# foolwood/SiamMask

Measured on AMD Instinct MI355X. Metric: frames/sec (255x255 search, 127x127 template), higher is better.
Workload: dtype f16; 1 GPU; siammask_sharp track_mask+track_refine, B=8 streams per GPU in lock-step, cached template; BASELINE configs[2]; variant=sharp, batch_per_gpu=8, global_batch=8, parallelism=streams sharded x1, weights=synthetic_damped (calibrated random init), graph=True, fallbacks=0

## Files before the change

siammask_amd/_lib.py:

```python
import ctypes
import os
import subprocess

import torch

_HERE = os.path.dirname(os.path.abspath(__file__))
LIB_PATH = os.environ.get("SMK_LIB") or os.path.join(_HERE, "libsiammask_hip.so")
CSRC = os.path.join(_HERE, "csrc")

DTYPE = {"f32": 0, "fp32": 0, "float32": 0, "f16": 1, "fp16": 1, "float16": 1, "half": 1,
         "f16x3": 2}
VARIANT = {"rpn": 0, "base": 1, "sharp": 2}
TRACK_BOX, TRACK_MASK, TRACK_NO_MASK_HEAD = 0, 1, 2
HP_STRIDE = 4

SYMBOLS = (
    "smk_version", "smk_last_error", "smk_create", "smk_destroy", "smk_set_weight",
    "smk_finalize_weights", "smk_template", "smk_track", "smk_refine", "smk_set_decode_params", "smk_decode", "smk_step", "smk_set_graph_mode", "smk_seq_status", "smk_seq_sync_check", "smk_set_result_ring", "smk_result_ring_cursor", "smk_set_pipeline", "smk_pipeline_join", "smk_pipeline_observe",
    "smk_debug_read", "smk_debug_seq_inject", "smk_tune", "smk_tune_get", "smk_profile", "smk_profile_dump", "smk_op_conv2d_ex", "smk_op_conv2d", "smk_op_dw_xcorr",
    "smk_op_maxpool3x3s2", "smk_op_stem_pool", "smk_op_l1_block", "smk_op_conv_seq", "smk_host_conv2d_ex", "smk_host_plan_conv", "smk_host_plan_seq", "smk_host_arena_elems", "smk_bench_conv", "smk_packed_size", "smk_export_packed",
    "smk_import_packed", "smk_crop_resize", "smk_paste_mask", "smk_paste_labels", "smk_mask_rbox_workspace", "smk_mask_rbox",
    "smk_trk_state_bytes", "smk_trk_set", "smk_trk_plan", "smk_trk_advance", "smk_crop_resize_dev", "smk_paste_mask_dev",
    "smk_vos_score", "smk_vos_score_dev", "smk_host_trk_plan", "smk_host_trk_advance",
    "smk_vos_score_ex", "smk_vos_score_dev_ex", "smk_label_rects", "smk_frame_sums", "smk_trk_start", "smk_crop_exemplar_dev",
    "smk_host_trk_start", "smk_vot_overlap", "smk_host_vot_overlap",
    "smk_crop_resize_dev_v", "smk_crop_exemplar_dev_v", "smk_frame_sums_v", "smk_trk_start_v", "smk_host_trk_start_v",
    "smk_paste_mask_dev_v", "smk_vot_overlap_dev",
    "smk_set_stream_hp", "smk_trk_advance_hp", "smk_host_trk_advance_hp",
    "smk_iou_score", "smk_iou_score_dev",
    "smk_mask_rbox_workspace_ex", "smk_mask_rbox_ex", "smk_test_mask_rbox_paths",
    "smk_rle_workspace", "smk_rle_encode", "smk_paste_rle_dev", "smk_test_rle_encode",
    "smk_paste_rle_dev_v", "smk_rle_encode_v", "smk_test_rle_encode_v",
    "smk_labels_rle_encode", "smk_vos_rle", "smk_vos_rle_dev",
    "smk_vos_rle_v", "smk_vos_rle_dev_v", "smk_vos_score_v", "smk_vos_score_dev_v",
    "smk_png_worst_bytes", "smk_png_workspace", "smk_png_encode", "smk_host_png_encode", "smk_vos_png_v", "smk_vos_png_dev_v",
# ... 83 lines not shown
    L.smk_tune_get.argtypes = [ctypes.c_char_p, ctypes.POINTER(ci)]
    L.smk_profile.argtypes = [vp, ci]
    L.smk_profile_dump.argtypes = [vp, ctypes.c_char_p, ci]
    ip = ctypes.POINTER(ci)
    L.smk_debug_read.argtypes = [vp, ctypes.c_char_p, fp, ip, ip, ip, vp]
    gp = ctypes.POINTER(ConvGeom)
    L.smk_op_conv2d_ex.argtypes = [ci, ci, gp, fp, fp, fp, fp, vp, fp, vp]
    L.smk_op_conv2d.argtypes = [ci, ci, fp, ci, ci, ci, ci, fp, fp, ci, ci, ci, ci, ci, ci, fp, fp, vp]
    L.smk_op_dw_xcorr.argtypes = [ci, fp, fp, ci, ci, ci, ci, ci, ci, fp, vp]
    L.smk_op_maxpool3x3s2.argtypes = [ci, fp, ci, ci, ci, ci, fp, vp]
    L.smk_op_stem_pool.argtypes = [fp, fp, fp, ci, ci, fp, fp, vp]
    L.smk_op_l1_block.argtypes = [fp] * 9 + [ci, ci, ci, fp, vp]
    L.smk_host_conv2d_ex.argtypes = [gp, fp, fp, fp, fp, vp, fp]
    L.smk_host_plan_conv.argtypes = [gp, ci, ci, ip, ip, ip, ip]
    L.smk_host_arena_elems.argtypes = [ci, ci, ci, ctypes.POINTER(ctypes.c_uint64)]
    L.smk_packed_size.argtypes = [vp, ctypes.POINTER(ctypes.c_uint64)]
    L.smk_export_packed.argtypes = [vp, vp, ctypes.c_uint64]
    L.smk_import_packed.argtypes = [vp, vp, ctypes.c_uint64]
    L.smk_crop_resize.argtypes = [vp, ctypes.c_int64, ci, ci, vp, vp, ci, ci, fp, vp]
    L.smk_paste_mask.argtypes = [fp, ci, vp, ci, ci, ci, ctypes.c_float, ctypes.c_float, vp, fp, vp]
    L.smk_paste_labels.argtypes = [fp, ci, vp, ci, ci, ci, ctypes.c_float, ctypes.c_float, vp, vp]
    L.smk_mask_rbox_workspace.argtypes = [ci, ci, ci]
    L.smk_mask_rbox.argtypes = [vp, ci, ci, ci, ctypes.c_double, vp, ctypes.c_size_t, vp, vp]
    L.smk_mask_rbox_workspace_ex.argtypes = [ci, ci, ci, ci]
    L.smk_mask_rbox_ex.argtypes = [vp, ci, ci, ci, ctypes.c_double, ci, vp, ctypes.c_size_t, vp, vp]
    L.smk_test_mask_rbox_paths.argtypes = [vp, ci, ci, ci, ci, vp]
    cp = ctypes.POINTER(TrkCfg)
    L.smk_trk_state_bytes.argtypes = [ci]
    L.smk_trk_set.argtypes = [vp, ci, vp, vp, vp, ci, ci, vp]
    L.smk_trk_plan.argtypes = [vp, ci, cp, vp]
# ... 108 lines not shown
```

siammask_amd/csrc/conv_igemm.hip:

```cpp
#include <hip/hip_runtime.h>
#include "smk_kernels.h"

namespace smk {

typedef _Float16 half8 __attribute__((ext_vector_type(8)));
typedef _Float16 half4 __attribute__((ext_vector_type(4)));
typedef float floatx16 __attribute__((ext_vector_type(16)));
typedef float floatx4 __attribute__((ext_vector_type(4)));

template <typename T> struct Traits;
template <> struct Traits<float> {
    static constexpr int VE = 4;
    typedef floatx4 frag_t;
    typedef floatx4 out4_t;
    static __device__ inline void mma(floatx16 &acc, const frag_t &a, const frag_t &b) {
        acc = __builtin_amdgcn_mfma_f32_32x32x2f32(a[0], b[0], acc, 0, 0, 0);
        acc = __builtin_amdgcn_mfma_f32_32x32x2f32(a[1], b[1], acc, 0, 0, 0);
        acc = __builtin_amdgcn_mfma_f32_32x32x2f32(a[2], b[2], acc, 0, 0, 0);
        acc = __builtin_amdgcn_mfma_f32_32x32x2f32(a[3], b[3], acc, 0, 0, 0);
    }
    static __device__ inline floatx4 load4(const float *p) { return *(const floatx4 *)p; }
    static __device__ inline void store4(float *p, floatx4 v) { *(floatx4 *)p = v; }
    static constexpr int EV = 4;
    static __device__ inline void loadv(const float *p, float (&v)[4]) {
// ... 826 lines not shown
    hipStream_t s = (hipStream_t)stream;
    const int ch = dtype == DT_F16 ? 64 : 32;
    if (!conv_halo_eligible(p, dtype, bm)) return 1;
    const int ch_n = p.Ci / ch;
    const long wgs64 = (long)p.B * ((p.Ho * p.Wo + 63) / 64) * ((p.Nst + 127) / 128);
    const bool db = bm == 64 && g_tune.halo_db && ch_n >= 2 && wgs64 <= 256;
    if (dtype == DT_F16) {
        if (bm == 128) return launch_halo_t<_Float16, 2, 2, 1, HALO_AROWS_128, 2, 1>(p, s);
        return db ? launch_halo_t<_Float16, 1, 2, 2, HALO_AROWS_64, 3, 2>(p, s) : launch_halo_t<_Float16, 1, 2, 2, HALO_AROWS_64, 3, 1>(p, s);
    }
    if (bm == 128) return launch_halo_t<float, 2, 2, 1, HALO_AROWS_128, 2, 1>(p, s);
    return db ? launch_halo_t<float, 1, 2, 2, HALO_AROWS_64, 3, 2>(p, s) : launch_halo_t<float, 1, 2, 2, HALO_AROWS_64, 3, 1>(p, s);
}

}
namespace smk {
#include "refine_chain_body.inc"
#include "mask_head_tile.inc"
constexpr int CM_CONV_LDS = IgemmLds<2, 2, 1, 128, 2>::v;
constexpr int CM_LDS = CMax<RC_LDS, 2 * CM_CONV_LDS>::v;
static_assert(MH_LDS <= CM_LDS, "the stationary-pixel mask-head tile fits the fused launch's LDS");

__global__ __launch_bounds__(1024) void chain_mask_kernel(const RefineChainParams rp, const ConvBatch cb, const int mh_nsplit) {
    __shared__ __attribute__((aligned(16))) unsigned char smem[CM_LDS];
    if ((int)blockIdx.x < rp.B) {
        refine_chain_body<false>(rp, (int)blockIdx.x, smem);
    } else if (mh_nsplit > 0) {
        mask_head_tile(cb.p[0], (int)blockIdx.x - rp.B, mh_nsplit, smem);
    } else {
        const int half = threadIdx.x >> 9;
        const int bx = 2 * ((int)blockIdx.x - rp.B) + half;
        if (bx < cb.start[cb.n])
            conv_igemm_body<_Float16, 2, 2, 1, 128, OUT_NCHW_F32, 2>(cb, bx, 0, half * 512, smem + half * CM_CONV_LDS);
    }
    if (rp.tail_sem) {
        __syncthreads();
        if (threadIdx.x == 0) {
            const unsigned prev = __hip_atomic_fetch_add(rp.tail_sem + 5, 1u, __ATOMIC_RELAXED, __HIP_MEMORY_SCOPE_AGENT);
            if (prev == gridDim.x - 1) {
                __hip_atomic_store(rp.tail_sem + 5, 0u, __ATOMIC_RELAXED, __HIP_MEMORY_SCOPE_AGENT);
                __hip_atomic_fetch_add(rp.tail_sem, 1u, __ATOMIC_RELEASE, __HIP_MEMORY_SCOPE_AGENT);
            }
        }
    }
}

// ... 5 lines not shown

bool mask_head_eligible(const ConvParams &p, int dtype) {
    return dtype == DT_F16 && p.out_mode == OUT_NCHW_F32 && p.wgt_frag != nullptr && p.kh == 1 && p.kw == 1 && p.stride == 1 &&
           p.stride_x == 1 && p.pad == 0 && !p.ups && !p.pos && p.org_y == 0 && p.org_x == 0 && p.Hl == p.Hs && p.Wl == p.Ws &&
           p.Ho == p.Hs && p.Wo == p.Ws && p.groups <= 1 && p.Ci == MH_K && p.K == MH_K && p.Kpad == MH_K && !p.relu &&
           !p.oscale && !p.x3_in && p.res_mode == RES_NONE && p.N >= 1 && p.N <= MH_NMAX && (p.Cs % 8) == 0 && (p.cin_off % 8) == 0 &&
           p.cin_off + MH_K <= p.Cs && p.M == p.B * p.Ho * p.Wo && p.in_bytes > 0 && p.in_bytes < 0x7fff0000u &&
           p.in_bytes >= (unsigned long long)p.M * p.Cs * 2 && p.w_bytes < 0x7fff0000u &&
           p.w_bytes >= (unsigned long long)((p.N + 31) / 32) * 32 * MH_K * 2 && (unsigned long long)p.M * p.N * 4 < 0x7fff0000ull;
}

int mask_head_nsplit(const ConvParams &p, int cus) {
    const int ptiles = (p.M + MH_PX - 1) / MH_PX, nblk = (p.N + 31) / 32;
    int cap = nblk / 8;
    if (cap < 1) cap = 1;
    if (ptiles * 2 <= cus) {
        const int ns = cus / ptiles;
        return ns < cap ? ns : cap;
    }
    int best = 1;
    double best_eff = 0.0;
    for (int ns = 2; ns <= 8 && ns <= cap; ++ns) {
        const long wgs = (long)ptiles * ns, rounds = (wgs + cus - 1) / cus;
        const double eff = (double)wgs / (double)(rounds * cus);
        if (eff > best_eff + 1e-9) { best_eff = eff; best = ns; }
    }
    return best;
}

static int mask_head_nt(const ConvParams &p) { return (p.nt_store && p.M <= 16 * 625) ? 1 : 0; }

int launch_mask_head(const ConvParams &p0, void *stream) {
    if (!mask_head_eligible(p0, DT_F16)) return 1;
    ConvParams p = p0;
    p.nt_store = mask_head_nt(p);
    const int nsplit = mask_head_nsplit(p, 256);
    const int ptiles = (p.M + MH_PX - 1) / MH_PX;
    hipLaunchKernelGGL(mask_head_kernel, dim3(ptiles * nsplit), dim3(1024), 0, (hipStream_t)stream, p, nsplit);
    return hipGetLastError() == hipSuccess ? 0 : -4;
}

int launch_chain_mask(const RefineChainParams &rp, ConvBatch &cb, int stationary, void *stream) {
    if (rp.v2_cs != 32 || rp.v1_cs != 16 || rp.v0_cs != 8 || cb.n != 1) return -1;
    ConvParams &p = cb.p[0];
    if (p.out_mode != OUT_NCHW_F32 || p.groups > 1) return -1;
    if (stationary && mask_head_eligible(p, DT_F16)) {
        const int nsplit = mask_head_nsplit(p, 256 - rp.B > 64 ? 256 - rp.B : 64);
        const int ptiles = (p.M + MH_PX - 1) / MH_PX;
        cb.start[0] = 0;
        for (int i = 1; i <= CONV_BATCH_MAX; ++i) cb.start[i] = ptiles * nsplit;
        p.ksplit = 1;
        p.nt_store = mask_head_nt(p);
        hipLaunchKernelGGL(chain_mask_kernel, dim3(rp.B + ptiles * nsplit), dim3(1024), 0, (hipStream_t)stream, rp, cb, nsplit);
        return hipGetLastError() == hipSuccess ? 0 : -4;
    }
    const int tiles = ((p.M + 127) / 128) * ((p.Nst + 127) / 128);
    if (tiles & 1) return 1;
    cb.start[0] = 0;
    for (int i = 1; i <= CONV_BATCH_MAX; ++i) cb.start[i] = tiles;
    p.ksplit = 1;
    hipLaunchKernelGGL(chain_mask_kernel, dim3(rp.B + (tiles + 1) / 2), dim3(1024), 0, (hipStream_t)stream, rp, cb, 0);
    return hipGetLastError() == hipSuccess ? 0 : -4;
}

template <typename T>
__global__ void conv_naive_kernel(const ConvParams p) {
    typedef Traits<T> TR;
    constexpr int VE = TR::VE;
    const int g = blockIdx.z;
    const int cin_off = p.cin_off + g * p.g_cin_off;
    const T *wgt = (const T *)p.wgt + (size_t)g * p.g_wgt_off * p.Kpad;
    const float *bias = p.bias + g * p.g_wgt_off;
    const int cout_off = p.cout_off + g * p.g_cout_off;
    const int nq = p.Nst / 4;
    const long total = (long)p.M * nq;
    const T *in = (const T *)p.in;
// ... 185 lines not shown
```

siammask_amd/csrc/engine.cpp:

```cpp
#include <hip/hip_runtime_api.h>

#include <cmath>
#include <cstdarg>
#include <tuple>
#include <cstdio>
#include <cstdlib>
#include <cstring>
#include <functional>
#include <map>
#include <memory>
#include <string>
#include <vector>

#include "../../include/siammask_hip.h"
#include "../../include/siammask_hip_test.h"
#include "engine_internal.h"

using namespace smk;

static thread_local std::string g_err;

namespace smk {
int fail(int code, const char *fmt, ...) {
    char buf[1024];
// ... 1030 lines not shown
        for (int i = 0; i < 9; ++i) {
            auto it = c->conv.find(ids[i]);
            if (it == c->conv.end()) return fail(SMK_E_STATE, "internal: conv %s not packed", ids[i]);
            const PackedConv &pc = it->second;
            if (pc.k != 3 || pc.groups != 1 || pc.Ci < geo[i][1] || pc.N != geo[i][2])
                return fail(SMK_E_STATE, "internal: conv %s does not have the Refine geometry", ids[i]);
            rp.L[i] = RefineChainLayer{pc.w, pc.bias, pc.Kpad, pc.Ci};
            flop += 2.0 * B * geo[i][0] * 9.0 * geo[i][1] * geo[i][2];
            wbytes += 2.0 * 9.0 * geo[i][1] * geo[i][2];
        }
        rp.d = d.p;
        rp.v2 = V2.p; rp.v1 = V1.p; rp.v0 = V0.p;
        rp.v2_cs = V2.C; rp.v1_cs = V1.C; rp.v0_cs = V0.C;
        rp.out = out;
        rp.B = B;
        rp.clk = nullptr;
        rp.ring = nullptr; rp.ring_cursor = nullptr; rp.ring_done = nullptr; rp.ring_rows = 0;
        rp.tail_sem = nullptr;
        if (rec.ring && c->ring_ref) {
            rp.ring = (_Float16 *)c->ring_ref; rp.ring_cursor = c->ring_cursor; rp.ring_done = (unsigned *)(c->ring_cursor + 1);
            rp.ring_rows = c->ring_rows;
            rec.ring_ref_folded = true;
        }
        static const bool want_clk = getenv("SMK_CHAIN_CLK") != nullptr;
        static unsigned long long *clk_dev = nullptr;
        hipStreamCaptureStatus cst = hipStreamCaptureStatusNone;
        if (want_clk && hipStreamIsCapturing(s, &cst) == hipSuccess && cst == hipStreamCaptureStatusNone) {
            if (!clk_dev) HIPCHK(hipMalloc((void **)&clk_dev, 32 * sizeof(unsigned long long)));
            rp.clk = clk_dev;
        }
// ... 921 lines not shown
```

siammask_amd/csrc/op_api.cpp:

```cpp
#include <cstdio>
#include <cstdlib>
#include <cstring>
#include <functional>
#include <string>
#include <vector>

#include "../../include/siammask_hip_test.h"
#include "engine_internal.h"

using namespace smk;

extern "C" {

struct TmpBufs {
    std::vector<void *> v;
    ~TmpBufs() { for (void *p : v) hipFree(p); }
    int alloc(void **p, size_t bytes) {
        HIPCHK(hipMalloc(p, bytes + 256));
        HIPCHK(hipMemset(*p, 0, bytes + 256));
        v.push_back(*p);
        return 0;
    }
};

// ... 673 lines not shown
    xin.H = ops[0].g.H; xin.W = ops[0].g.W; xin.C = rup(ops[0].g.Cin, 8); xin.p = tensors;
    int next = 1;
    std::vector<SeqRec> rec;
    std::vector<Act> outs;
    CHK(seq_op_records(ops, n, xin, -1, [](int, PackedConv &pc) { fake_pack(pc, DT_F16); return 0; },
                       [&](void **p, size_t) { *p = tensors + next++; return 0; }, rec, outs));
    plan_seq_ops(ops, rec, outs, grid);
    for (int i = 0; i < n; ++i) {
        cfg[i] = rec[i].L.cfg;
        sync[i] = rec[i].L.sync;
        a_stage[i] = rec[i].L.a_stage;
    }
    return 0;
}

}
```

siammask_amd/csrc/refine_chain.hip:

```cpp
#include <hip/hip_runtime.h>

#include "smk_kernels.h"

namespace smk {

#include "refine_chain_body.inc"

template <bool TIMED>
__global__ __launch_bounds__(1024) void refine_chain_kernel(const RefineChainParams p) {
    __shared__ __attribute__((aligned(16))) unsigned char smem[RC_LDS];
    refine_chain_body<TIMED>(p, (int)blockIdx.x, smem);
}

int launch_refine_chain(const RefineChainParams &p, void *stream) {
    if (p.v2_cs != 32 || p.v1_cs != 16 || p.v0_cs != 8) return -1;
    if (p.clk) hipLaunchKernelGGL(refine_chain_kernel<true>, dim3(p.B), dim3(RC_NT), 0, (hipStream_t)stream, p);
    else hipLaunchKernelGGL(refine_chain_kernel<false>, dim3(p.B), dim3(RC_NT), 0, (hipStream_t)stream, p);
    return hipGetLastError() == hipSuccess ? 0 : -4;
}

}
```

siammask_amd/csrc/refine_chain_body.inc:

```
typedef _Float16 half8 __attribute__((ext_vector_type(8)));
typedef _Float16 half4 __attribute__((ext_vector_type(4)));
typedef _Float16 half2v __attribute__((ext_vector_type(2)));
typedef float floatx4 __attribute__((ext_vector_type(4)));

namespace {

constexpr int RC_NT = 1024;
constexpr int RC_BUF = 33 * 33 * 16 * 2;
constexpr int RC_WROWS = 32, RC_WPITCH = 288 + 8;
constexpr int RC_WSTAGE = RC_WROWS * RC_WPITCH * 2 + RC_WROWS * 4;
constexpr int RC_TAB = 132;
constexpr int RC_LDS = 3 * RC_BUF + 2 * RC_WSTAGE + 2 * RC_TAB * 4;

__device__ __forceinline__ void lds_barrier() {
    asm volatile("s_waitcnt lgkmcnt(0)" ::: "memory");
    __builtin_amdgcn_s_barrier();
    asm volatile("" ::: "memory");
}

template <int CIN, int COUT>
struct WGeo {
    static constexpr int K = 9 * CIN, KSTEPS = (K + 31) / 32, KP = KSTEPS * 32 + 8, NT = (COUT + 15) / 16;
    static constexpr int G = KSTEPS * 8;
    static constexpr int TOTAL = NT * 16 * G, PER = (TOTAL + RC_NT - 1) / RC_NT;
// ... 77 lines not shown
    }
}

template <int H, int C>
__device__ __forceinline__ void zero_image(_Float16 *img) {
    constexpr int N16 = ((H + 2) * (H + 2) * C * 2 + 15) / 16;
    const floatx4 z = {0.f, 0.f, 0.f, 0.f};
    for (int i = threadIdx.x; i < N16; i += RC_NT) ((floatx4 *)img)[i] = z;
}

template <int CIN, int COUT, int H, int SRC, bool RELU, bool RES, bool OUT_GLOBAL, int NCIN, int NCOUT, int FCIN,
          int FCOUT, int VH, int VC>
__device__ __forceinline__ void chain_layer(const _Float16 *in, _Float16 *out, const _Float16 *wl, _Float16 *wl_next,
                                            const WR<NCIN, NCOUT> &wnext, const RefineChainLayer &Lfar,
                                            WR<FCIN, FCOUT> &wfar, const _Float16 *vsrc, _Float16 *vimg,
                                            const int *tab, float *gout) {
    typedef WGeo<CIN, COUT> WG;
    constexpr int KSTEPS = WG::KSTEPS, KP = WG::KP, NT = WG::NT, M = H * H, MT = (M + 15) / 16;
    constexpr int HI = SRC > 0 ? SRC : H, W2 = HI + 2;
    constexpr int WO = H + 2;
    constexpr bool PRELOAD = KSTEPS * NT <= 10;
    const int tid = threadIdx.x, lane = tid & 63, wave = tid >> 6;

    VRegs<VH ? VH : 1, VH ? VC : 8> vn;
    if (FCIN) w_load<FCIN ? FCIN : 4, FCIN ? FCOUT : 1>(Lfar, wfar);
    if (VH) v_load<VH ? VH : 1, VH ? VC : 8>(vsrc, vn);
    if (!OUT_GLOBAL && !RES) zero_image<H, COUT>(out);
    if (VH) zero_image<VH ? VH : 1, VH ? VC : 8>(vimg);
    if (SRC > 0) build_up_tables<H, (SRC > 0 ? SRC : 1), CIN>((int *)tab);
    lds_barrier();

    const int fr = lane & 15, kq = lane >> 4;
    floatx4 bias4[NT];
// ... 8 lines not shown
        const int c0 = k0 - tap * CIN;
        tap = tap > 8 ? 8 : tap;
        kh_[ks] = (tap * 11) >> 5;
        kw_[ks] = tap - 3 * kh_[ks];
        koff[ks] = SRC > 0 ? c0 : (kh_[ks] * W2 + kw_[ks]) * CIN + c0;
    }
    half8 wf[PRELOAD ? KSTEPS : 1][NT];
    if (PRELOAD) {
#pragma unroll
        for (int ks = 0; ks < KSTEPS; ++ks)
#pragma unroll
            for (int nt = 0; nt < NT; ++nt) wf[ks][nt] = *(const half8 *)(wl + (nt * 16 + fr) * KP + ks * 32 + kq * 8);
    }

    for (int mt = wave; mt < MT; mt += RC_NT / 64) {
        int m = mt * 16 + fr;
        m = m < M ? m : M - 1;
        const int oy = m / H, ox = m - oy * H;
        const int pbase = (oy * W2 + ox) * CIN;
        auto a_off = [&](int ks) {
            if (SRC > 0) return tab[oy + kh_[ks]] + tab[RC_TAB + ox + kw_[ks]] + koff[ks];
            return pbase + koff[ks];
        };
        floatx4 acc[NT];
#pragma unroll
        for (int nt = 0; nt < NT; ++nt) acc[nt] = floatx4{0.f, 0.f, 0.f, 0.f};
#pragma unroll
        for (int ks = 0; ks < KSTEPS; ++ks) {
            const half8 a = *(const half8 *)(in + a_off(ks));
#pragma unroll
            for (int nt = 0; nt < NT; ++nt) {
                const half8 b = PRELOAD ? wf[PRELOAD ? ks : 0][nt]
                                        : *(const half8 *)(wl + (nt * 16 + fr) * KP + ks * 32 + kq * 8);
                acc[nt] = __builtin_amdgcn_mfma_f32_16x16x32_f16(b, a, acc[nt], 0, 0, 0);
            }
        }
        const bool px_ok = mt * 16 + fr < M;
#pragma unroll
        for (int nt = 0; nt < NT; ++nt) {
            const int n = nt * 16 + 4 * kq;
            if (OUT_GLOBAL) {
                if (n == 0 && px_ok) gout[mt * 16 + fr] = acc[nt][0] + bias4[nt][0];
            } else if (n < COUT && px_ok) {
                static_assert(OUT_GLOBAL || COUT % 4 == 0, "four channels per lane");
                _Float16 *o = out + ((oy + 1) * WO + ox + 1) * COUT + n;
                float v[4];
#pragma unroll
                for (int i = 0; i < 4; ++i) {
                    v[i] = acc[nt][i] + bias4[nt][i];
                    if (RELU) v[i] = fmaxf(v[i], 0.f);
                }
                if (RES) {
                    const half4 r = *(const half4 *)o;
#pragma unroll
                    for (int i = 0; i < 4; ++i) v[i] += (float)r[i];
                }
                *(half4 *)o = half4{(_Float16)v[0], (_Float16)v[1], (_Float16)v[2], (_Float16)v[3]};
            }
        }
    }
    if (NCIN) w_store<NCIN ? NCIN : 4, NCIN ? NCOUT : 1>(wl_next, wnext);
    if (VH) v_store<VH ? VH : 1, VH ? VC : 8>(vimg, vn);
    lds_barrier();
}

template <int COUT, int H, int SRC, bool RELU, bool RES, bool OUT_GLOBAL, int NCIN, int NCOUT, int FCIN, int FCOUT,
          int VH, int VC>
__device__ __forceinline__ void chain_layer_c4(const _Float16 *in, _Float16 *out, const _Float16 *wl, _Float16 *wl_next,
                                               const WR<NCIN, NCOUT> &wnext, const RefineChainLayer &Lfar,
                                               WR<FCIN, FCOUT> &wfar, const _Float16 *vsrc, _Float16 *vimg,
                                               const int *tab, float *gout, _Float16 *gout16 = nullptr) {
    typedef WGeo<4, COUT> WG;
    constexpr int KP = WG::KP, M = H * H;
    constexpr int HI = SRC > 0 ? SRC : H, W2 = HI + 2, WO = H + 2;
    static_assert(COUT == 4 || COUT == 1, "output channels");
    const int tid = threadIdx.x;

    VRegs<VH ? VH : 1, VH ? VC : 8> vn;
    if (FCIN) w_load<FCIN ? FCIN : 4, FCIN ? FCOUT : 1>(Lfar, wfar);
    if (VH) v_load<VH ? VH : 1, VH ? VC : 8>(vsrc, vn);
    if (!OUT_GLOBAL && !RES) zero_image<H, COUT>(out);
    if (VH) zero_image<VH ? VH : 1, VH ? VC : 8>(vimg);
    if (SRC > 0) build_up_tables<H, (SRC > 0 ? SRC : 1), 4>((int *)tab);
    lds_barrier();

    half2v wv[COUT][9][2];
    float bias[COUT];
#pragma unroll
    for (int co = 0; co < COUT; ++co) {
        bias[co] = ((const float *)(wl + RC_WROWS * RC_WPITCH))[co];
#pragma unroll
        for (int t = 0; t < 9; ++t) {
            const half4 w4 = *(const half4 *)(wl + co * KP + t * 4);
            wv[co][t][0] = half2v{w4[0], w4[1]};
            wv[co][t][1] = half2v{w4[2], w4[3]};
        }
    }
    for (int px = tid; px < M; px += RC_NT) {
        const int oy = px / H, ox = px - oy * H;
        float acc[COUT];
#pragma unroll
        for (int co = 0; co < COUT; ++co) acc[co] = 0.f;
        if (SRC > 0) {
            int ro[3], cl[3];
#pragma unroll
            for (int t = 0; t < 3; ++t) {
                ro[t] = tab[oy + t];
                cl[t] = tab[RC_TAB + ox + t];
            }
#pragma unroll
            for (int t = 0; t < 9; ++t) {
                const half4 a = *(const half4 *)(in + ro[t / 3] + cl[t % 3]);
#pragma unroll
// ... 35 lines not shown
                *(half4 *)o = half4{(_Float16)v[0], (_Float16)v[COUT > 1 ? 1 : 0], (_Float16)v[COUT > 2 ? 2 : 0],
                                    (_Float16)v[COUT > 3 ? 3 : 0]};
            } else {
                *o = (_Float16)v[0];
            }
        }
    }
    if (NCIN) w_store<NCIN ? NCIN : 4, NCIN ? NCOUT : 1>(wl_next, wnext);
    if (VH) v_store<VH ? VH : 1, VH ? VC : 8>(vimg, vn);
    lds_barrier();
}

}

template <bool TIMED>
__device__ __forceinline__ void refine_chain_body(const RefineChainParams &p, const int b, unsigned char *smem) {
    _Float16 *bA = (_Float16 *)smem, *bB = (_Float16 *)(smem + RC_BUF), *bC = (_Float16 *)(smem + 2 * RC_BUF);
    _Float16 *w0 = (_Float16 *)(smem + 3 * RC_BUF), *w1 = (_Float16 *)(smem + 3 * RC_BUF + RC_WSTAGE);
    const _Float16 *v2 = (const _Float16 *)p.v2 + (size_t)b * (225 * 32);
    const _Float16 *v1 = (const _Float16 *)p.v1 + (size_t)b * (961 * 16);
    const _Float16 *v0 = (const _Float16 *)p.v0 + (size_t)b * (3721 * 8);
    float *gout = p.out + (size_t)b * (127 * 127);
    _Float16 *gout16 = nullptr;
    if (p.ring) gout16 = p.ring + ((size_t)(*(volatile const unsigned *)p.ring_cursor % (unsigned)p.ring_rows) * p.B + b) * (127 * 127);
    int *tab = (int *)(smem + 3 * RC_BUF + 2 * RC_WSTAGE);
    unsigned long long *clk = TIMED && p.clk && b == 0 && threadIdx.x == 0 ? p.clk : nullptr;
    if (TIMED && clk) clk[0] = wall_clock64();
    WRegs<32, 32> r1;
    WRegs<32, 16> r2;
    WRegs<16, 16> r3, r4;
    WRegs<16, 4> r5;
    WRegs<4, 4> r6, r7;
    WRegs<4, 1> r8, none;
    {
        WRegs<32, 32> r0;
        VRegs<15, 32> dr;
        w_load<32, 32>(p.L[0], r0);
        v_load<15, 32>((const _Float16 *)p.d + (size_t)b * 7200, dr);
        w_load<32, 32>(p.L[1], r1);
        zero_image<15, 32>(bA);
        lds_barrier();
        w_store<32, 32>(w0, r0);
        v_store<15, 32>(bA, dr);
    }
    if (TIMED && clk) clk[1] = wall_clock64();
    chain_layer<32, 32, 15, 0, true, false, false, 32, 32, 32, 16, 15, 32>(bA, bB, w0, w1, r1, p.L[2], r2, v2, bC, tab, nullptr);
    if (TIMED && clk) clk[2] = wall_clock64();
    chain_layer<32, 32, 15, 0, true, true, false, 32, 16, 16, 16, 0, 0>(bB, bC, w1, w0, r2, p.L[3], r3, nullptr, nullptr, tab, nullptr);
    if (TIMED && clk) clk[3] = wall_clock64();
    chain_layer<32, 16, 31, 15, false, false, false, 16, 16, 16, 16, 0, 0>(bC, bA, w0, w1, r3, p.L[4], r4, nullptr, nullptr, tab, nullptr);
    if (TIMED && clk) clk[4] = wall_clock64();
    chain_layer<16, 16, 31, 0, true, false, false, 16, 16, 16, 4, 31, 16>(bA, bB, w1, w0, r4, p.L[5], r5, v1, bC, tab, nullptr);
    if (TIMED && clk) clk[5] = wall_clock64();
    chain_layer<16, 16, 31, 0, true, true, false, 16, 4, 4, 4, 0, 0>(bB, bC, w0, w1, r5, p.L[6], r6, nullptr, nullptr, tab, nullptr);
    if (TIMED && clk) clk[6] = wall_clock64();
    chain_layer<16, 4, 61, 31, false, false, false, 4, 4, 4, 4, 0, 0>(bC, bA, w1, w0, r6, p.L[7], r7, nullptr, nullptr, tab, nullptr);
    if (TIMED && clk) clk[7] = wall_clock64();
    chain_layer_c4<4, 61, 0, true, false, false, 4, 4, 4, 1, 61, 4>(bA, bB, w0, w1, r7, p.L[8], r8, v0, bC, tab, nullptr);
    if (TIMED && clk) clk[8] = wall_clock64();
    chain_layer_c4<4, 61, 0, true, true, false, 4, 1, 0, 0, 0, 0>(bB, bC, w1, w0, r8, p.L[8], none, nullptr, nullptr, tab, nullptr);
    if (TIMED && clk) clk[9] = wall_clock64();
    chain_layer_c4<1, 127, 61, false, false, true, 0, 0, 0, 0, 0, 0>(bC, nullptr, w0, nullptr, none, p.L[8], none, nullptr, nullptr, tab, gout, gout16);
    if (TIMED && clk) clk[10] = wall_clock64();
    if (p.ring && threadIdx.x == 0) {
        const unsigned prev = __hip_atomic_fetch_add(p.ring_done, 1u, __ATOMIC_RELAXED, __HIP_MEMORY_SCOPE_AGENT);
        if (prev == (unsigned)p.B - 1) {
            __hip_atomic_store(p.ring_done, 0u, __ATOMIC_RELAXED, __HIP_MEMORY_SCOPE_AGENT);
            __hip_atomic_fetch_add(p.ring_cursor, 1, __ATOMIC_RELAXED, __HIP_MEMORY_SCOPE_AGENT);
        }
    }
}
```

siammask_amd/csrc/smk_kernels.h:

```cpp
#pragma once
#include <stdint.h>

#if defined(__HIPCC__)
#define SMK_HD __host__ __device__ inline
#else
#define SMK_HD inline
#endif

namespace smk {

enum { DT_F32 = 0, DT_F16 = 1, DT_F16X3 = 2 };
enum { RES_NONE = 0, RES_PRE_RELU = 1, RES_POST_RELU = 2 };
enum { OUT_NHWC = 0, OUT_NCHW_F32 = 1 };

constexpr int NPAD_ALIGN = 128;
constexpr int KPAD_ALIGN = 128;

struct ConvParams {
    const void *in;
    const void *wgt;
    const void *wgt_frag;
    const void *wgt_frag_halo;
    const float *bias;
    const void *res;
// ... 100 lines not shown
    SeqLayer L[SEQ_MAX];
};
static_assert(sizeof(SeqArgs) <= 4096, "the layer list travels in the kernel-argument segment");

struct Tuning {
    int xcd_mode = 1;
    int force_tile = 0;
    int min_blocks_x16 = 16;
    int stages = 0;
    int kt = 0;
    int prio = 0;
    int nt_store = 1;
    int halo = 1;
    int halo_db = 1;
    int chain = 1;
    int ksplit = 0;
    int xc_ch = 64;
    int l1_fused = 1;
    int stem_fused = 1;
    int xc_full = 0;
    int buf_lds = 1;
    int chain_mask = 1;
    int nchw_tn_major = 1;
    int merge = 1;
    int merge_max_batch = 32;
    int rf_wreg = 3;
    int seq_fuse3 = 0;
    int seq_spoll = 1;
    int wreg = 1;
    int wreg_stages = 0;
    int seq = 1;
    int seq_min_batch = 5, seq_max_batch = 8;
    int seq_extra_batch = 12;
    int seq_mult_max = 24;
    int ablate = 0;
    int seq_tall = 2;
    int seq_kstag = 1;
// ... 175 lines not shown
int launch_conv_pair(const SeqLayer &L3, const SeqLayer &L1, int code, int M, void *stream, int rows);
int conv_seq_occupancy();
int xcc_census(int grid, int *out_host);
struct RefineChainLayer {
    const void *w;
    const float *bias;
    int Kpad, Ci;
};
struct RefineChainParams {
    const void *d;
    const void *v2, *v1, *v0;
    int v2_cs, v1_cs, v0_cs;
    RefineChainLayer L[9];
    float *out;
    int B;
    unsigned long long *clk;
    _Float16 *ring;
    int *ring_cursor;
    unsigned *ring_done;
    int ring_rows;
    unsigned *tail_sem;
};
int launch_refine_chain(const RefineChainParams &p, void *stream);
int launch_chain_mask(const RefineChainParams &rp, ConvBatch &cb, int stationary, void *stream);
bool mask_head_eligible(const ConvParams &p, int dtype);
int mask_head_nsplit(const ConvParams &p, int cus);
int launch_mask_head(const ConvParams &p, void *stream);
int launch_xcorr(const XcorrParams &p, int dtype, void *stream);
int launch_xcorr_x3(const XcorrParams &p, void *stream);
void xcorr_prepare();
// ... 50 lines not shown
```

siammask_amd/csrc/tune.cpp:

```cpp
#include <cstdlib>
#include <cstring>

#include "../../include/siammask_hip_test.h"
#include "engine_internal.h"

using namespace smk;

extern "C" {

enum { KNOB_RAW = 0, KNOB_BOOL = -1 };
struct Knob { const char *name; int *slot; const char *accept; int conv; const char *product; };
#ifdef SMK_MEASURE
static int g_measure_build = 1;
#else
static int g_measure_build = 0;
#endif
static const Knob KNOBS[] = {
    {"xcd_mode", &g_tune.xcd_mode, "*", KNOB_RAW, nullptr},
    {"force_tile", &g_tune.force_tile, "0..5", KNOB_RAW, nullptr},
    {"min_blocks_x16", &g_tune.min_blocks_x16, "*", KNOB_RAW, nullptr},
    {"stages", &g_tune.stages, "0|2..4", KNOB_RAW, nullptr},
    {"kt", &g_tune.kt, "0|128|256", KNOB_RAW, nullptr},
    {"prio", &g_tune.prio, "-1..3", KNOB_RAW, nullptr},
    {"nt_store", &g_tune.nt_store, "*", KNOB_BOOL, nullptr},
// ... 40 lines not shown
    {"seq_yres", &g_tune.seq_yres, "*", KNOB_BOOL, nullptr},
    {"seq_search", &g_tune.seq_search, "*", KNOB_BOOL, nullptr},
    {"seq_first_stage", &g_tune.seq_first_stage, "0..3", KNOB_RAW, "1..3"},
    {"seq_min_batch", &g_tune.seq_min_batch, ">=1", KNOB_RAW, nullptr},
    {"seq_max_batch", &g_tune.seq_max_batch, ">=1", KNOB_RAW, nullptr},
    {"seq_extra_batch", &g_tune.seq_extra_batch, "*", KNOB_RAW, nullptr},
    {"seq_mult_max", &g_tune.seq_mult_max, ">=0", KNOB_RAW, nullptr},
    {"main_prio", &g_tune.main_prio, "0..3", KNOB_RAW, nullptr},
    {"pipe_late", &g_tune.pipe_late, "*", KNOB_BOOL, nullptr},
    {"seq_fused_last", &g_seq_last.pairs, nullptr, KNOB_RAW, nullptr},
    {"seq_yres_last", &g_seq_last.resident, nullptr, KNOB_RAW, nullptr},
    {"seq_fused3_last", &g_seq_last.triples, nullptr, KNOB_RAW, nullptr},
    {"measure_build", &g_measure_build, nullptr, KNOB_RAW, nullptr},
};

static bool knob_accepts(const char *spec, int v) {
    if (!strcmp(spec, "*")) return true;
    for (const char *t = spec; t; t = strchr(t, '|') ? strchr(t, '|') + 1 : nullptr) {
        if (t[0] == '>' && t[1] == '=') {
            if (v >= atoi(t + 2)) return true;
            continue;
        }
        char *e = nullptr;
        const long lo = strtol(t, &e, 10), hi = (e[0] == '.' && e[1] == '.') ? strtol(e + 2, nullptr, 10) : lo;
        if (v >= lo && v <= hi) return true;
    }
    return false;
}

static const Knob *find_knob(const char *key) {
    for (const Knob &k : KNOBS)
        if (!strcmp(key, k.name)) return &k;
    return nullptr;
}

int smk_tune(const char *key, int value) {
    if (!key) return fail(SMK_E_ARG, "smk_tune: key is NULL");
    const Knob *k = find_knob(key);
    if (!k) return fail(SMK_E_ARG, "smk_tune: unknown key %s", key);
    if (!k->accept) return fail(SMK_E_ARG, "smk_tune: %s is a read-only diagnostic", key);
    if (!knob_accepts(k->accept, value)) return fail(SMK_E_ARG, "smk_tune: %s takes %s, not %d", key, k->accept, value);
#ifndef SMK_MEASURE
    if (k->product && !knob_accepts(k->product, value))
        return fail(SMK_E_ARG, "smk_tune: %s %d is a measured alternative, only in a library built with `make MEASURE=1` (this one takes %s)",
                    key, value, k->product);
#endif
// ... 16 lines not shown
```

Measured before the change: 16110 frames/sec.

## Split refine chain tail layers into row bands across multiple workgroups per stream

The refine chain kernel used one workgroup per batch item. It now launches B*S workgroups, where S is 1, 2 or 4 and is picked from the batch size and CU count, so S is 4 for B=8. Each band recomputes the early layers and then computes only its halo-padded rows of the 61x61 and 127x127 tail layers. This aims to spread the long serial tail across more CUs, at the cost of redundant front-layer work and more LDS-heavy workgroups. The mask-head split count also gets a fixed 80-workgroup target when the shared tail semaphore is used, and there is a new tuning knob for it.

```diff
diff --git a/siammask_amd/_lib.py b/siammask_amd/_lib.py
--- a/siammask_amd/_lib.py
+++ b/siammask_amd/_lib.py
@@ -18,7 +18,7 @@
     "smk_version", "smk_last_error", "smk_create", "smk_destroy", "smk_set_weight",
     "smk_finalize_weights", "smk_template", "smk_track", "smk_refine", "smk_set_decode_params", "smk_decode", "smk_step", "smk_set_graph_mode", "smk_seq_status", "smk_seq_sync_check", "smk_set_result_ring", "smk_result_ring_cursor", "smk_set_pipeline", "smk_pipeline_join", "smk_pipeline_observe",
     "smk_debug_read", "smk_debug_seq_inject", "smk_tune", "smk_tune_get", "smk_profile", "smk_profile_dump", "smk_op_conv2d_ex", "smk_op_conv2d", "smk_op_dw_xcorr",
-    "smk_op_maxpool3x3s2", "smk_op_stem_pool", "smk_op_l1_block", "smk_op_conv_seq", "smk_host_conv2d_ex", "smk_host_plan_conv", "smk_host_plan_seq", "smk_host_arena_elems", "smk_bench_conv", "smk_packed_size", "smk_export_packed",
+    "smk_op_maxpool3x3s2", "smk_op_stem_pool", "smk_op_l1_block", "smk_op_conv_seq", "smk_host_conv2d_ex", "smk_host_plan_conv", "smk_host_plan_seq", "smk_host_arena_elems", "smk_host_chain_rows", "smk_bench_conv", "smk_packed_size", "smk_export_packed",
     "smk_import_packed", "smk_crop_resize", "smk_paste_mask", "smk_paste_labels", "smk_mask_rbox_workspace", "smk_mask_rbox",
     "smk_trk_state_bytes", "smk_trk_set", "smk_trk_plan", "smk_trk_advance", "smk_crop_resize_dev", "smk_paste_mask_dev",
     "smk_vos_score", "smk_vos_score_dev", "smk_host_trk_plan", "smk_host_trk_advance",
@@ -132,6 +132,7 @@
     L.smk_host_conv2d_ex.argtypes = [gp, fp, fp, fp, fp, vp, fp]
     L.smk_host_plan_conv.argtypes = [gp, ci, ci, ip, ip, ip, ip]
     L.smk_host_arena_elems.argtypes = [ci, ci, ci, ctypes.POINTER(ctypes.c_uint64)]
+    L.smk_host_chain_rows.argtypes = [ci, ci, ip]
     L.smk_packed_size.argtypes = [vp, ctypes.POINTER(ctypes.c_uint64)]
     L.smk_export_packed.argtypes = [vp, vp, ctypes.c_uint64]
     L.smk_import_packed.argtypes = [vp, vp, ctypes.c_uint64]
diff --git a/siammask_amd/csrc/chain_rows.h b/siammask_amd/csrc/chain_rows.h
--- /dev/null
+++ b/siammask_amd/csrc/chain_rows.h
@@ -0,0 +1,39 @@
+#pragma once
+
+#if defined(__HIPCC__) || defined(__CUDACC__)
+#define SMK_CHAIN_HD __host__ __device__ inline
+#else
+#define SMK_CHAIN_HD inline
+#endif
+
+namespace smk {
+
+constexpr int CHAIN_H_FINE = 127, CHAIN_H_MID = 61;
+
+struct ChainRows {
+    int post1[2], h00[2], h02[2], post2[2];
+};
+
+SMK_CHAIN_HD constexpr bool chain_split_valid(int S) { return S == 1 || S == 2 || S == 4; }
+
+SMK_CHAIN_HD constexpr ChainRows chain_rows(int S, int s) {
+    ChainRows r{};
+    r.post2[0] = s * CHAIN_H_FINE / S;
+    r.post2[1] = (s + 1) * CHAIN_H_FINE / S;
+    const int lo = r.post2[0] > 0 ? r.post2[0] - 1 : 0;
+    const int hi = r.post2[1] < CHAIN_H_FINE ? r.post2[1] : CHAIN_H_FINE - 1;
+    r.h02[0] = lo * CHAIN_H_MID / CHAIN_H_FINE;
+    r.h02[1] = hi * CHAIN_H_MID / CHAIN_H_FINE + 1;
+    r.h00[0] = r.h02[0] > 0 ? r.h02[0] - 1 : 0;
+    r.h00[1] = r.h02[1] < CHAIN_H_MID ? r.h02[1] + 1 : CHAIN_H_MID;
+    r.post1[0] = r.h00[0] > 0 ? r.h00[0] - 1 : 0;
+    r.post1[1] = r.h00[1] < CHAIN_H_MID ? r.h00[1] + 1 : CHAIN_H_MID;
+    return r;
+}
+
+SMK_CHAIN_HD constexpr int chain_split_rule(int B, int cus, int forced) {
+    if (chain_split_valid(forced)) return forced;
+    return B * 4 <= cus ? 4 : (B * 2 <= cus ? 2 : 1);
+}
+
+}
diff --git a/siammask_amd/csrc/conv_igemm.hip b/siammask_amd/csrc/conv_igemm.hip
--- a/siammask_amd/csrc/conv_igemm.hip
+++ b/siammask_amd/csrc/conv_igemm.hip
@@ -864,6 +864,7 @@
 }
 
 }
+#include "chain_rows.h"
 namespace smk {
 #include "refine_chain_body.inc"
 #include "mask_head_tile.inc"
@@ -873,13 +874,14 @@
 
 __global__ __launch_bounds__(1024) void chain_mask_kernel(const RefineChainParams rp, const ConvBatch cb, const int mh_nsplit) {
     __shared__ __attribute__((aligned(16))) unsigned char smem[CM_LDS];
-    if ((int)blockIdx.x < rp.B) {
+    const int chain_wgs = rp.B * rp.S;
+    if ((int)blockIdx.x < chain_wgs) {
         refine_chain_body<false>(rp, (int)blockIdx.x, smem);
     } else if (mh_nsplit > 0) {
-        mask_head_tile(cb.p[0], (int)blockIdx.x - rp.B, mh_nsplit, smem);
+        mask_head_tile(cb.p[0], (int)blockIdx.x - chain_wgs, mh_nsplit, smem);
     } else {
         const int half = threadIdx.x >> 9;
-        const int bx = 2 * ((int)blockIdx.x - rp.B) + half;
+        const int bx = 2 * ((int)blockIdx.x - chain_wgs) + half;
         if (bx < cb.start[cb.n])
             conv_igemm_body<_Float16, 2, 2, 1, 128, OUT_NCHW_F32, 2>(cb, bx, 0, half * 512, smem + half * CM_CONV_LDS);
     }
@@ -915,6 +917,7 @@
     const int ptiles = (p.M + MH_PX - 1) / MH_PX, nblk = (p.N + 31) / 32;
     int cap = nblk / 8;
     if (cap < 1) cap = 1;
+    if (g_tune.mask_nsplit > 0) return g_tune.mask_nsplit < cap ? g_tune.mask_nsplit : cap;
     if (ptiles * 2 <= cus) {
         const int ns = cus / ptiles;
         return ns < cap ? ns : cap;
@@ -927,6 +930,16 @@
         if (eff > best_eff + 1e-9) { best_eff = eff; best = ns; }
     }
     return best;
+}
+
+constexpr int MH_SHARED_WGS = 80;
+static int mask_head_nsplit_shared(const ConvParams &p) {
+    const int ptiles = (p.M + MH_PX - 1) / MH_PX, nblk = (p.N + 31) / 32;
+    int cap = nblk / 8;
+    if (cap < 1) cap = 1;
+    if (g_tune.mask_nsplit > 0) return g_tune.mask_nsplit < cap ? g_tune.mask_nsplit : cap;
+    const int ns = (MH_SHARED_WGS + ptiles - 1) / ptiles;
+    return ns < cap ? ns : cap;
 }
 
 static int mask_head_nt(const ConvParams &p) { return (p.nt_store && p.M <= 16 * 625) ? 1 : 0; }
@@ -941,18 +954,21 @@
     return hipGetLastError() == hipSuccess ? 0 : -4;
 }
 
-int launch_chain_mask(const RefineChainParams &rp, ConvBatch &cb, int stationary, void *stream) {
-    if (rp.v2_cs != 32 || rp.v1_cs != 16 || rp.v0_cs != 8 || cb.n != 1) return -1;
+int launch_chain_mask(const RefineChainParams &rp0, ConvBatch &cb, int stationary, void *stream) {
+    if (rp0.v2_cs != 32 || rp0.v1_cs != 16 || rp0.v0_cs != 8 || cb.n != 1 || rp0.B < 1) return -1;
     ConvParams &p = cb.p[0];
     if (p.out_mode != OUT_NCHW_F32 || p.groups > 1) return -1;
+    RefineChainParams rp = rp0;
+    rp.S = chain_split_rule(rp.B, 256, g_tune.chain_split);
+    const int chain_wgs = rp.B * rp.S;
     if (stationary && mask_head_eligible(p, DT_F16)) {
-        const int nsplit = mask_head_nsplit(p, 256 - rp.B > 64 ? 256 - rp.B : 64);
+        const int nsplit = rp.tail_sem ? mask_head_nsplit_shared(p) : mask_head_nsplit(p, 256 - chain_wgs > 64 ? 256 - chain_wgs : 64);
         const int ptiles = (p.M + MH_PX - 1) / MH_PX;
         cb.start[0] = 0;
         for (int i = 1; i <= CONV_BATCH_MAX; ++i) cb.start[i] = ptiles * nsplit;
         p.ksplit = 1;
         p.nt_store = mask_head_nt(p);
-        hipLaunchKernelGGL(chain_mask_kernel, dim3(rp.B + ptiles * nsplit), dim3(1024), 0, (hipStream_t)stream, rp, cb, nsplit);
+        hipLaunchKernelGGL(chain_mask_kernel, dim3(chain_wgs + ptiles * nsplit), dim3(1024), 0, (hipStream_t)stream, rp, cb, nsplit);
         return hipGetLastError() == hipSuccess ? 0 : -4;
     }
     const int tiles = ((p.M + 127) / 128) * ((p.Nst + 127) / 128);
@@ -960,7 +976,7 @@
     cb.start[0] = 0;
     for (int i = 1; i <= CONV_BATCH_MAX; ++i) cb.start[i] = tiles;
     p.ksplit = 1;
-    hipLaunchKernelGGL(chain_mask_kernel, dim3(rp.B + (tiles + 1) / 2), dim3(1024), 0, (hipStream_t)stream, rp, cb, 0);
+    hipLaunchKernelGGL(chain_mask_kernel, dim3(chain_wgs + (tiles + 1) / 2), dim3(1024), 0, (hipStream_t)stream, rp, cb, 0);
     return hipGetLastError() == hipSuccess ? 0 : -4;
 }
 
diff --git a/siammask_amd/csrc/engine.cpp b/siammask_amd/csrc/engine.cpp
--- a/siammask_amd/csrc/engine.cpp
+++ b/siammask_amd/csrc/engine.cpp
@@ -1068,6 +1068,7 @@
         rp.v2_cs = V2.C; rp.v1_cs = V1.C; rp.v0_cs = V0.C;
         rp.out = out;
         rp.B = B;
+        rp.S = 0;
         rp.clk = nullptr;
         rp.ring = nullptr; rp.ring_cursor = nullptr; rp.ring_done = nullptr; rp.ring_rows = 0;
         rp.tail_sem = nullptr;
diff --git a/siammask_amd/csrc/op_api.cpp b/siammask_amd/csrc/op_api.cpp
--- a/siammask_amd/csrc/op_api.cpp
+++ b/siammask_amd/csrc/op_api.cpp
@@ -6,6 +6,7 @@
 #include <vector>
 
 #include "../../include/siammask_hip_test.h"
+#include "chain_rows.h"
 #include "engine_internal.h"
 
 using namespace smk;
@@ -711,4 +712,15 @@
     return 0;
 }
 
-}
+int smk_host_chain_rows(int S, int s, int out[8]) {
+    if (!out) return fail(SMK_E_ARG, "smk_host_chain_rows: null argument");
+    if (!chain_split_valid(S) || s < 0 || s >= S) return fail(SMK_E_ARG, "smk_host_chain_rows: band %d of %d (1, 2 or 4 bands)", s, S);
+    const ChainRows r = chain_rows(S, s);
+    out[0] = r.post1[0]; out[1] = r.post1[1];
+    out[2] = r.h00[0]; out[3] = r.h00[1];
+    out[4] = r.h02[0]; out[5] = r.h02[1];
+    out[6] = r.post2[0]; out[7] = r.post2[1];
+    return 0;
+}
+
+}
diff --git a/siammask_amd/csrc/refine_chain.hip b/siammask_amd/csrc/refine_chain.hip
--- a/siammask_amd/csrc/refine_chain.hip
+++ b/siammask_amd/csrc/refine_chain.hip
@@ -1,5 +1,6 @@
 #include <hip/hip_runtime.h>
 
+#include "chain_rows.h"
 #include "smk_kernels.h"
 
 namespace smk {
@@ -12,10 +13,12 @@
     refine_chain_body<TIMED>(p, (int)blockIdx.x, smem);
 }
 
-int launch_refine_chain(const RefineChainParams &p, void *stream) {
-    if (p.v2_cs != 32 || p.v1_cs != 16 || p.v0_cs != 8) return -1;
-    if (p.clk) hipLaunchKernelGGL(refine_chain_kernel<true>, dim3(p.B), dim3(RC_NT), 0, (hipStream_t)stream, p);
-    else hipLaunchKernelGGL(refine_chain_kernel<false>, dim3(p.B), dim3(RC_NT), 0, (hipStream_t)stream, p);
+int launch_refine_chain(const RefineChainParams &p0, void *stream) {
+    if (p0.v2_cs != 32 || p0.v1_cs != 16 || p0.v0_cs != 8 || p0.B < 1) return -1;
+    RefineChainParams p = p0;
+    p.S = chain_split_rule(p.B, 256, g_tune.chain_split);
+    if (p.clk) hipLaunchKernelGGL(refine_chain_kernel<true>, dim3(p.B * p.S), dim3(RC_NT), 0, (hipStream_t)stream, p);
+    else hipLaunchKernelGGL(refine_chain_kernel<false>, dim3(p.B * p.S), dim3(RC_NT), 0, (hipStream_t)stream, p);
     return hipGetLastError() == hipSuccess ? 0 : -4;
 }
 
diff --git a/siammask_amd/csrc/refine_chain_body.inc b/siammask_amd/csrc/refine_chain_body.inc
--- a/siammask_amd/csrc/refine_chain_body.inc
+++ b/siammask_amd/csrc/refine_chain_body.inc
@@ -115,9 +115,10 @@
 __device__ __forceinline__ void chain_layer(const _Float16 *in, _Float16 *out, const _Float16 *wl, _Float16 *wl_next,
                                             const WR<NCIN, NCOUT> &wnext, const RefineChainLayer &Lfar,
                                             WR<FCIN, FCOUT> &wfar, const _Float16 *vsrc, _Float16 *vimg,
-                                            const int *tab, float *gout) {
+                                            const int *tab, float *gout, const int y0 = 0, const int y1 = H) {
     typedef WGeo<CIN, COUT> WG;
-    constexpr int KSTEPS = WG::KSTEPS, KP = WG::KP, NT = WG::NT, M = H * H, MT = (M + 15) / 16;
+    constexpr int KSTEPS = WG::KSTEPS, KP = WG::KP, NT = WG::NT;
+    const int M0 = y0 * H, M = y1 * H, MT = (M - M0 + 15) / 16;
     constexpr int HI = SRC > 0 ? SRC : H, W2 = HI + 2;
     constexpr int WO = H + 2;
     constexpr bool PRELOAD = KSTEPS * NT <= 10;
@@ -156,7 +157,7 @@
     }
 
     for (int mt = wave; mt < MT; mt += RC_NT / 64) {
-        int m = mt * 16 + fr;
+        int m = M0 + mt * 16 + fr;
         m = m < M ? m : M - 1;
         const int oy = m / H, ox = m - oy * H;
         const int pbase = (oy * W2 + ox) * CIN;
@@ -177,12 +178,12 @@
                 acc[nt] = __builtin_amdgcn_mfma_f32_16x16x32_f16(b, a, acc[nt], 0, 0, 0);
             }
         }
-        const bool px_ok = mt * 16 + fr < M;
+        const bool px_ok = M0 + mt * 16 + fr < M;
 #pragma unroll
         for (int nt = 0; nt < NT; ++nt) {
             const int n = nt * 16 + 4 * kq;
             if (OUT_GLOBAL) {
-                if (n == 0 && px_ok) gout[mt * 16 + fr] = acc[nt][0] + bias4[nt][0];
+                if (n == 0 && px_ok) gout[M0 + mt * 16 + fr] = acc[nt][0] + bias4[nt][0];
             } else if (n < COUT && px_ok) {
                 static_assert(OUT_GLOBAL || COUT % 4 == 0, "four channels per lane");
                 _Float16 *o = out + ((oy + 1) * WO + ox + 1) * COUT + n;
@@ -211,9 +212,10 @@
 __device__ __forceinline__ void chain_layer_c4(const _Float16 *in, _Float16 *out, const _Float16 *wl, _Float16 *wl_next,
                                                const WR<NCIN, NCOUT> &wnext, const RefineChainLayer &Lfar,
                                                WR<FCIN, FCOUT> &wfar, const _Float16 *vsrc, _Float16 *vimg,
-                                               const int *tab, float *gout, _Float16 *gout16 = nullptr) {
+                                               const int *tab, float *gout, _Float16 *gout16, const int y0, const int y1) {
     typedef WGeo<4, COUT> WG;
-    constexpr int KP = WG::KP, M = H * H;
+    constexpr int KP = WG::KP;
+    const int M0 = y0 * H, M = y1 * H;
     constexpr int HI = SRC > 0 ? SRC : H, W2 = HI + 2, WO = H + 2;
     static_assert(COUT == 4 || COUT == 1, "output channels");
     const int tid = threadIdx.x;
@@ -238,7 +240,7 @@
             wv[co][t][1] = half2v{w4[2], w4[3]};
         }
     }
-    for (int px = tid; px < M; px += RC_NT) {
+    for (int px = M0 + tid; px < M; px += RC_NT) {
         const int oy = px / H, ox = px - oy * H;
         float acc[COUT];
 #pragma unroll
@@ -304,7 +306,9 @@
 }
 
 template <bool TIMED>
-__device__ __forceinline__ void refine_chain_body(const RefineChainParams &p, const int b, unsigned char *smem) {
+__device__ __forceinline__ void refine_chain_body(const RefineChainParams &p, const int wg, unsigned char *smem) {
+    const int s = wg / p.B, b = wg - s * p.B;
+    const ChainRows R = chain_rows(p.S, s);
     _Float16 *bA = (_Float16 *)smem, *bB = (_Float16 *)(smem + RC_BUF), *bC = (_Float16 *)(smem + 2 * RC_BUF);
     _Float16 *w0 = (_Float16 *)(smem + 3 * RC_BUF), *w1 = (_Float16 *)(smem + 3 * RC_BUF + RC_WSTAGE);
     const _Float16 *v2 = (const _Float16 *)p.v2 + (size_t)b * (225 * 32);
@@ -314,7 +318,7 @@
     _Float16 *gout16 = nullptr;
     if (p.ring) gout16 = p.ring + ((size_t)(*(volatile const unsigned *)p.ring_cursor % (unsigned)p.ring_rows) * p.B + b) * (127 * 127);
     int *tab = (int *)(smem + 3 * RC_BUF + 2 * RC_WSTAGE);
-    unsigned long long *clk = TIMED && p.clk && b == 0 && threadIdx.x == 0 ? p.clk : nullptr;
+    unsigned long long *clk = TIMED && p.clk && wg == 0 && threadIdx.x == 0 ? p.clk : nullptr;
     if (TIMED && clk) clk[0] = wall_clock64();
     WRegs<32, 32> r1;
     WRegs<32, 16> r2;
@@ -344,17 +348,17 @@
     if (TIMED && clk) clk[5] = wall_clock64();
     chain_layer<16, 16, 31, 0, true, true, false, 16, 4, 4, 4, 0, 0>(bB, bC, w0, w1, r5, p.L[6], r6, nullptr, nullptr, tab, nullptr);
     if (TIMED && clk) clk[6] = wall_clock64();
-    chain_layer<16, 4, 61, 31, false, false, false, 4, 4, 4, 4, 0, 0>(bC, bA, w1, w0, r6, p.L[7], r7, nullptr, nullptr, tab, nullptr);
+    chain_layer<16, 4, 61, 31, false, false, false, 4, 4, 4, 4, 0, 0>(bC, bA, w1, w0, r6, p.L[7], r7, nullptr, nullptr, tab, nullptr, R.post1[0], R.post1[1]);
     if (TIMED && clk) clk[7] = wall_clock64();
-    chain_layer_c4<4, 61, 0, true, false, false, 4, 4, 4, 1, 61, 4>(bA, bB, w0, w1, r7, p.L[8], r8, v0, bC, tab, nullptr);
+    chain_layer_c4<4, 61, 0, true, false, false, 4, 4, 4, 1, 61, 4>(bA, bB, w0, w1, r7, p.L[8], r8, v0, bC, tab, nullptr, nullptr, R.h00[0], R.h00[1]);
     if (TIMED && clk) clk[8] = wall_clock64();
-    chain_layer_c4<4, 61, 0, true, true, false, 4, 1, 0, 0, 0, 0>(bB, bC, w1, w0, r8, p.L[8], none, nullptr, nullptr, tab, nullptr);
+    chain_layer_c4<4, 61, 0, true, true, false, 4, 1, 0, 0, 0, 0>(bB, bC, w1, w0, r8, p.L[8], none, nullptr, nullptr, tab, nullptr, nullptr, R.h02[0], R.h02[1]);
     if (TIMED && clk) clk[9] = wall_clock64();
-    chain_layer_c4<1, 127, 61, false, false, true, 0, 0, 0, 0, 0, 0>(bC, nullptr, w0, nullptr, none, p.L[8], none, nullptr, nullptr, tab, gout, gout16);
+    chain_layer_c4<1, 127, 61, false, false, true, 0, 0, 0, 0, 0, 0>(bC, nullptr, w0, nullptr, none, p.L[8], none, nullptr, nullptr, tab, gout, gout16, R.post2[0], R.post2[1]);
     if (TIMED && clk) clk[10] = wall_clock64();
     if (p.ring && threadIdx.x == 0) {
         const unsigned prev = __hip_atomic_fetch_add(p.ring_done, 1u, __ATOMIC_RELAXED, __HIP_MEMORY_SCOPE_AGENT);
-        if (prev == (unsigned)p.B - 1) {
+        if (prev == (unsigned)(p.B * p.S) - 1) {
             __hip_atomic_store(p.ring_done, 0u, __ATOMIC_RELAXED, __HIP_MEMORY_SCOPE_AGENT);
             __hip_atomic_fetch_add(p.ring_cursor, 1, __ATOMIC_RELAXED, __HIP_MEMORY_SCOPE_AGENT);
         }
diff --git a/siammask_amd/csrc/smk_kernels.h b/siammask_amd/csrc/smk_kernels.h
--- a/siammask_amd/csrc/smk_kernels.h
+++ b/siammask_amd/csrc/smk_kernels.h
@@ -138,6 +138,7 @@
     int halo = 1;
     int halo_db = 1;
     int chain = 1;
+    int chain_split = 0;
     int ksplit = 0;
     int xc_ch = 64;
     int l1_fused = 1;
@@ -145,6 +146,7 @@
     int xc_full = 0;
     int buf_lds = 1;
     int chain_mask = 1;
+    int mask_nsplit = 0;
     int nchw_tn_major = 1;
     int merge = 1;
     int merge_max_batch = 32;
@@ -350,6 +352,7 @@
     RefineChainLayer L[9];
     float *out;
     int B;
+    int S;
     unsigned long long *clk;
     _Float16 *ring;
     int *ring_cursor;
diff --git a/siammask_amd/csrc/tune.cpp b/siammask_amd/csrc/tune.cpp
--- a/siammask_amd/csrc/tune.cpp
+++ b/siammask_amd/csrc/tune.cpp
@@ -78,6 +78,11 @@
     {"measure_build", &g_measure_build, nullptr, KNOB_RAW, nullptr},
 };
 
+static const Knob TAIL_KNOBS[] = {
+    {"chain_split", &g_tune.chain_split, "0|1|2|4", KNOB_RAW, nullptr},
+    {"mask_nsplit", &g_tune.mask_nsplit, "0..15", KNOB_RAW, nullptr},
+};
+
 static bool knob_accepts(const char *spec, int v) {
     if (!strcmp(spec, "*")) return true;
     for (const char *t = spec; t; t = strchr(t, '|') ? strchr(t, '|') + 1 : nullptr) {
@@ -94,6 +99,8 @@
 
 static const Knob *find_knob(const char *key) {
     for (const Knob &k : KNOBS)
+        if (!strcmp(key, k.name)) return &k;
+    for (const Knob &k : TAIL_KNOBS)
         if (!strcmp(key, k.name)) return &k;
     return nullptr;
 }
```

Measured after the change: 16570 frames/sec, median of 6. +2.8%, better.
